# thomasdeppisch/eMagLS

Hardware: AMD Instinct MI355X
Metric: eMagLS filter sets/s (N=4, 2702 dirs, 512 taps) (higher is better)
Workload: dtype f64; 1 GPU; BASELINE config 3: getEMagLsFilters em32 r=4.2cm N=4 complex-SH, 2702 dirs, 512 taps, 48 kHz; one filter set per step, inputs resident in HBM; dirs=2702, taps=512, sim_order=19, bins=512, k_cut=43, designs_resident_per_gpu=128, designs_per_batch=32, batches_in_flight=4, distinct_hrir_sets_resident=20, parallelism=independent jobs per GPU, one RCCL gather

## Files before the change

### emagls_amd/csrc/fft.hip

```cpp
#include "kernels.hpp"
#include "lds_fft.hpp"
#include "wave_fft.hpp"

namespace emagls {

__global__ void twiddle_kernel(int nfft, cplx* __restrict__ tw, size_t bstride) {
    tw = boff(tw, bstride);
    int j = blockIdx.x * blockDim.x + threadIdx.x;
    if (j >= nfft) return;
    double s, c;
    sincos(-2.0 * kPi * (double)j / (double)nfft, &s, &c);
    if (j == 0) { c = 1.0; s = 0.0; }
    if (2 * j == nfft) { c = -1.0; s = 0.0; }
    if (4 * j == nfft) { c = 0.0; s = -1.0; }
    if (4 * j == 3 * nfft) { c = 0.0; s = 1.0; }
    tw[j] = mk(c, s);
}

__global__ void __launch_bounds__(256) hrir_dirsum_kernel(const double* __restrict__ hL, const double* __restrict__ hR,
                                                          int64_t L, int64_t D, int chunk, double* __restrict__ partial, size_t bstride) {
    hL = boff(hL, bstride); hR = boff(hR, bstride); partial = boff(partial, bstride);
    const int e = blockIdx.y;
    const double* h = e ? hR : hL;
    const int64_t d0 = (int64_t)blockIdx.x * chunk;
    const int64_t d1 = min(D, d0 + chunk);
    for (int64_t n = threadIdx.x; n < L; n += blockDim.x) {
        double acc = 0.0;
        for (int64_t d = d0; d < d1; ++d) acc += h[d * L + n];
        partial[((int64_t)blockIdx.x * 2 + e) * L + n] = acc;
    }
}

__global__ void __launch_bounds__(1024) grpdelay_median_kernel(const double* __restrict__ partial, int nchunks, int64_t L,
                                                               int nfft, const cplx* __restrict__ tw,
                                                               double* __restrict__ grpd, size_t bstride) {
    partial = boff(partial, bstride); tw = boff(tw, bstride); grpd = boff(grpd, bstride);
    extern __shared__ __attribute__((aligned(16))) char smem[];
    double* b = reinterpret_cast<double*>(smem);
    double* v = b + ((L + 1) & ~(int64_t)1);
    const int e = blockIdx.x;
    const int P = nfft / 2 + 1;
    int npow2 = 1;
    while (npow2 < P) npow2 <<= 1;
    {
        double* part = reinterpret_cast<double*>(reinterpret_cast<cplx*>(v + npow2) + nfft);
        const int nq = (int)max((int64_t)1, min((int64_t)8, (int64_t)blockDim.x / max(L, (int64_t)1)));
        for (int64_t idx = threadIdx.x; idx < (int64_t)nq * L; idx += blockDim.x) {
            const int64_t n = idx % L;
            const int q = (int)(idx / L);
            double a0 = 0.0, a1 = 0.0, a2 = 0.0, a3 = 0.0;
            int c = q;
            for (; c + 3 * nq < nchunks; c += 4 * nq) {
                a0 += partial[((int64_t)c * 2 + e) * L + n];
                a1 += partial[((int64_t)(c + nq) * 2 + e) * L + n];
                a2 += partial[((int64_t)(c + 2 * nq) * 2 + e) * L + n];
                a3 += partial[((int64_t)(c + 3 * nq) * 2 + e) * L + n];
            }
            for (; c < nchunks; c += nq) a0 += partial[((int64_t)c * 2 + e) * L + n];
            part[idx] = (a0 + a1) + (a2 + a3);
        }
        __syncthreads();
        for (int64_t n = threadIdx.x; n < L; n += blockDim.x) {
            double acc = 0.0;
            for (int q = 0; q < nq; ++q) acc += part[(int64_t)q * L + n];
            b[n] = acc;
        }
    }
    __syncthreads();
    cplx* tws = reinterpret_cast<cplx*>(v + npow2);
    for (int j = threadIdx.x; j < nfft; j += blockDim.x) tws[j] = tw[j];
    __syncthreads();
    auto finish = [](cplx num, cplx den) {
        if (cabs(den) < 10.0 * 2.220446049250313e-16) { num = mk(0, 0); den = mk(1, 0); }
        return cdiv(num, den).x;
    };
    const int kmain = min(P, (int)blockDim.x);
    for (int k = threadIdx.x; k < npow2; k += blockDim.x) v[k] = INFINITY;
    if ((int)threadIdx.x < kmain) {
        const int k = threadIdx.x;
        cplx num = mk(0, 0), den = mk(0, 0);
        int j = 0;
        for (int64_t n = 0; n < L; ++n) {
            const cplx w = tws[j];
            j += k; if (j >= nfft) j -= nfft;
            cfma(den, b[n], w);
            cfma(num, (double)n * b[n], w);
        }
        v[k] = finish(num, den);
    }
    for (int k = kmain; k < P; ++k) {
        __shared__ double red[16];
        cplx num = mk(0, 0), den = mk(0, 0);
        for (int64_t n = threadIdx.x; n < L; n += blockDim.x) {
            const cplx w = tws[(int)(((int64_t)k * n) % nfft)];
            cfma(den, b[n], w);
            cfma(num, (double)n * b[n], w);
        }
        double parts[4] = {num.x, num.y, den.x, den.y};
        for (int q = 0; q < 4; ++q) {
            double x = wave_sum(parts[q]);
            __syncthreads();
            if ((threadIdx.x & 63) == 0) red[threadIdx.x >> 6] = x;
            __syncthreads();
            double t = 0.0;
            for (int w = 0; w < (int)(blockDim.x >> 6); ++w) t += red[w];
            parts[q] = t;
        }
        if (threadIdx.x == 0) v[k] = finish(mk(parts[0], parts[1]), mk(parts[2], parts[3]));
    }
    __syncthreads();
    for (int size = 2; size <= npow2; size <<= 1) {
        for (int stride = size >> 1; stride > 0; stride >>= 1) {
            for (int i = threadIdx.x; i < npow2 / 2; i += blockDim.x) {
                const int lo = ((i / stride) * 2 * stride) + (i % stride);
                const int hi = lo + stride;
                const bool up = ((lo & size) == 0);
                const double a = v[lo], c = v[hi];
                if ((a > c) == up) { v[lo] = c; v[hi] = a; }
            }
            __syncthreads();
        }
    }
    const double med = (P & 1) ? v[(P - 1) / 2] : 0.5 * (v[P / 2 - 1] + v[P / 2]);
    if (threadIdx.x == 0) grpd[e] = med;
    cplx* phs = reinterpret_cast<cplx*>(grpd + 2) + (size_t)e * P;
    for (int kb = threadIdx.x; kb < P; kb += blockDim.x) {
        double sn, cs;
        sincos((6.283185307179586 * ((double)kb / (double)nfft)) * med, &sn, &cs);
        if (kb == P - 1) sn = 0.0;
        phs[kb] = mk(cs, sn);
    }
}

constexpr int HF_TD = 8;
constexpr int HF_MAXS = 3;
template <int TS>
__global__ void __launch_bounds__(512) hrir_fft_kernel(const double* __restrict__ hL, const double* __restrict__ hR,
                                                       int64_t L, int64_t D, const int64_t* __restrict__ didx, int nfft,
                                                       int log2n,
                                                       const cplx* __restrict__ tw, const double* __restrict__ grpd,
                                                       int mode, int n_c, int kabs0, cplx* __restrict__ Hc,
                                                       double* __restrict__ Habs, int64_t ldD, double* __restrict__ HcT, int ldT,
                                                       size_t bstride) {
    hL = boff(hL, bstride); hR = boff(hR, bstride); didx = boff(didx, bstride); tw = boff(tw, bstride); grpd = boff(grpd, bstride); Hc = boff(Hc, bstride); Habs = boff(Habs, bstride);
    HcT = boff(HcT, bstride);
    extern __shared__ __attribute__((aligned(16))) char smem[];
    const int P = nfft / 2 + 1;
    cplx* tws = reinterpret_cast<cplx*>(smem);
    cplx* phs = tws;
    cplx* buf = tws + 2 * P;
    const int64_t d0 = (int64_t)blockIdx.x * HF_TD;
    const int nt = (int)min((int64_t)HF_TD, D - d0);
// ... 47 lines not shown
            if (kb < P) {
#pragma unroll
                for (int t = 0; t < TS; ++t) {
                    if (t < nts) {
                        const cplx* x = buf + (size_t)t * nfft;
                        const cplx z = x[kb], zc = conj(x[(nfft - kb) & (nfft - 1)]);
                        cplx HLv = mk(0.5 * (z.x + zc.x), 0.5 * (z.y + zc.y));
                        cplx HRv = mk(0.5 * (z.y - zc.y), -0.5 * (z.x - zc.x));
                        if (mode == 0) {
                            HLv = HLv * phs[kb];
                            HRv = HRv * phs[P + kb];
                        }
                        if (!live[2 * (t0 + t)]) HLv = mk(0.0, 0.0);
                        if (!live[2 * (t0 + t) + 1]) HRv = mk(0.0, 0.0);
                        const int64_t d = d0 + t0 + t;
                        if (kb < n_c) {
                            Hc[((int64_t)0 * n_c + kb) * ldD + d] = HLv;
                            Hc[((int64_t)1 * n_c + kb) * ldD + d] = HRv;
                        }
                        const double nl2 = norm2(HLv), nr2 = norm2(HRv);
                        habs[s][0][t0 + t] = nl2 > 0.0 ? nl2 * fast_rsqrt(nl2) : 0.0;
                        habs[s][1][t0 + t] = nr2 > 0.0 ? nr2 * fast_rsqrt(nr2) : 0.0;
                    }
                }
            }
        }
        if (HcT) {
            for (int idx = threadIdx.x; idx < TS * n_c; idx += blockDim.x) {
                const int t = idx / n_c, kb = idx - t * n_c;
                if (t >= nts) continue;
                const cplx* x = buf + (size_t)t * nfft;
                const cplx z = x[kb], zc = conj(x[(nfft - kb) & (nfft - 1)]);
                cplx HLv = mk(0.5 * (z.x + zc.x), 0.5 * (z.y + zc.y));
                cplx HRv = mk(0.5 * (z.y - zc.y), -0.5 * (z.x - zc.x));
                if (mode == 0) { HLv = HLv * phs[kb]; HRv = HRv * phs[P + kb]; }
                if (!live[2 * (t0 + t)]) HLv = mk(0.0, 0.0);
                if (!live[2 * (t0 + t) + 1]) HRv = mk(0.0, 0.0);
                double* row = HcT + (int64_t)(d0 + t0 + t) * ldT;
                row[2 * kb] = HLv.x; row[2 * kb + 1] = HLv.y;
                row[2 * (n_c + kb)] = HRv.x; row[2 * (n_c + kb) + 1] = HRv.y;
            }
        }
    }
    const int64_t na = P - kabs0;
#pragma unroll
    for (int s = 0; s < HF_MAXS; ++s) {
        const int kb = threadIdx.x + s * 512;
        if (kb < P && kb >= kabs0) {
#pragma unroll
            for (int e = 0; e < 2; ++e) {
                double* row = Habs + ((int64_t)e * na + (kb - kabs0)) * ldD + d0;
                if (nt == HF_TD) {
#pragma unroll
                    for (int t = 0; t < HF_TD; t += 2) *reinterpret_cast<double2*>(row + t) = make_double2(habs[s][e][t], habs[s][e][t + 1]);
                } else {
#pragma unroll
                    for (int t = 0; t < HF_TD; ++t) if (t < nt) row[t] = habs[s][e][t];
                }
            }
        }
    }
}

constexpr int HW_TD = 8;
constexpr int HW_STRIDE = WF_BUF + 1;
__global__ void __launch_bounds__(64 * HW_TD) hrir_fft_wave_kernel(const double* __restrict__ hL, const double* __restrict__ hR,
                                                                   int64_t L, int64_t D, const int64_t* __restrict__ didx,
                                                                   const cplx* __restrict__ tw, const double* __restrict__ grpd,
                                                                   int mode, int n_c, int kabs0, cplx* __restrict__ Hc,
                                                                   double* __restrict__ Habs, int64_t ldD, double* __restrict__ HcT, int ldT,
                                                                   size_t bstride) {
    hL = boff(hL, bstride); hR = boff(hR, bstride); didx = boff(didx, bstride); tw = boff(tw, bstride); grpd = boff(grpd, bstride); Hc = boff(Hc, bstride); Habs = boff(Habs, bstride);
    HcT = boff(HcT, bstride);
    extern __shared__ __attribute__((aligned(16))) char smem[];
    constexpr int P = WF_N / 2 + 1;
    cplx* tables = reinterpret_cast<cplx*>(smem);
    cplx* bufs = tables + WF_TABLES;
    const int tid = threadIdx.x, w = tid >> 6, l = tid & 63;
    wave_fft_tables(tables, tw, tid, 64 * HW_TD);
    __syncthreads();
    const int64_t d0 = (int64_t)blockIdx.x * HW_TD;
    const int nt = (int)min((int64_t)HW_TD, D - d0);
    cplx* tb = bufs + (size_t)w * HW_STRIDE;
    if (w < nt) {
        const int64_t d = d0 + w;
        const int64_t dsrc = didx ? didx[d] : d;
        const double* pl = hL + dsrc * L;
        const double* pr = hR + dsrc * L;
        cplx v[16];
        const bool upper_zero = mode == 0 && L <= WF_N / 2;
        if (mode == 0) {
#pragma unroll
            for (int n1 = 0; n1 < 16; ++n1) {
                const int n = 64 * n1 + l;
                v[n1] = (n < L && (n1 < 8 || !upper_zero)) ? mk(pl[n], pr[n]) : mk(0.0, 0.0);
            }
        } else {
            const int sL = (int)round(grpd[0]), sR = (int)round(grpd[1]);
#pragma unroll
            for (int n1 = 0; n1 < 16; ++n1) {
                const int n = 64 * n1 + l;
                int nl = (n + sL) % WF_N; if (nl < 0) nl += WF_N;
                int nr = (n + sR) % WF_N; if (nr < 0) nr += WF_N;
                v[n1] = mk(nl < L ? pl[nl] : 0.0, nr < L ? pr[nr] : 0.0);
            }
        }
        bool nzL = false, nzR = false;
#pragma unroll
        for (int n1 = 0; n1 < 16; ++n1) { nzL |= v[n1].x != 0.0; nzR |= v[n1].y != 0.0; }
        const bool liveL = __any(nzL), liveR = __any(nzR);
        if (upper_zero) wave_fft1024<true>(v, tb, tables, l); else wave_fft1024<false>(v, tb, tables, l);
        wave_fft_store_natural(v, tb, l);
        wave_lds_fence();
        const cplx* phs = reinterpret_cast<const cplx*>(grpd + 2);
#pragma unroll
        for (int s = 0; s < 9; ++s) {
            const int kb = l + 64 * s;
            if (kb < P) {
                const cplx z = tb[wf_slot(kb)], zc = conj(tb[wf_slot((WF_N - kb) & (WF_N - 1))]);
                cplx HLv = mk(0.5 * (z.x + zc.x), 0.5 * (z.y + zc.y));
                cplx HRv = mk(0.5 * (z.y - zc.y), -0.5 * (z.x - zc.x));
                if (mode == 0) {
                    HLv = HLv * phs[kb];
                    HRv = HRv * phs[P + kb];
                }
                if (!liveL) HLv = mk(0.0, 0.0);
                if (!liveR) HRv = mk(0.0, 0.0);
                if (kb < n_c) {
                    Hc[((int64_t)0 * n_c + kb) * ldD + d] = HLv;
                    Hc[((int64_t)1 * n_c + kb) * ldD + d] = HRv;
                    if (HcT) {
                        double* rowT = HcT + d * ldT;
                        *reinterpret_cast<cplx*>(rowT + 2 * kb) = HLv;
                        *reinterpret_cast<cplx*>(rowT + 2 * (n_c + kb)) = HRv;
                    }
                }
                const double nl2 = norm2(HLv), nr2 = norm2(HRv);
                tb[wf_slot(kb)] = mk(nl2 > 0.0 ? nl2 * fast_rsqrt(nl2) : 0.0, nr2 > 0.0 ? nr2 * fast_rsqrt(nr2) : 0.0);
            }
        }
    }
    __syncthreads();
    const int64_t na = P - kabs0;
    const int t = tid & (HW_TD - 1);
    if (t < nt) {
        const double* src = reinterpret_cast<const double*>(bufs + (size_t)t * HW_STRIDE);
        for (int idx = tid >> 3; idx < 2 * (P - kabs0); idx += 64) {
            const int e = idx >= P - kabs0, kr = idx - e * (P - kabs0);
            Habs[((int64_t)e * na + kr) * ldD + d0 + t] = src[2 * wf_slot(kr + kabs0) + e];
        }
    }
}

__global__ void __launch_bounds__(512) real_fft_gather_kernel(const double* __restrict__ x, int64_t L, int64_t ncols,
                                                              const int64_t* __restrict__ colidx, int nfft, int log2n,
                                                              int TP, const cplx* __restrict__ tw,
                                                              cplx* __restrict__ out, int64_t ldo, int64_t inner,
                                                              int64_t ld_inner) {
    extern __shared__ __attribute__((aligned(16))) char smem[];
    cplx* tws = reinterpret_cast<cplx*>(smem);
    cplx* buf = tws + nfft / 2;
    const int P = nfft / 2 + 1;
    const int64_t p0 = (int64_t)blockIdx.x * TP;
    const int64_t npairs = (ncols + 1) / 2;
    const int nt = (int)min((int64_t)TP, npairs - p0);
    for (int j = threadIdx.x; j < nfft / 2; j += blockDim.x) tws[j] = tw[j];
    for (int idx = threadIdx.x; idx < nt * nfft; idx += blockDim.x) {
        const int t = idx / nfft, n = idx - t * nfft;
        const int64_t j0 = 2 * (p0 + t), j1 = j0 + 1;
        double a = 0.0, c = 0.0;
        if (n < L) {
            a = x[(colidx ? colidx[j0] : j0) * L + n];
            if (j1 < ncols) c = x[(colidx ? colidx[j1] : j1) * L + n];
        }
        buf[(size_t)t * nfft + bitrev((unsigned)n, log2n)] = mk(a, c);
    }
    __syncthreads();
    lds_fft_stages<false>(buf, tws, nfft, log2n, nt);
    for (int idx = threadIdx.x; idx < P * 2 * TP; idx += blockDim.x) {
        const int kb = idx / (2 * TP), r = idx - kb * 2 * TP;
        const int t = r >> 1, which = r & 1;
        if (t >= nt) continue;
        const int64_t j = 2 * (p0 + t) + which;
        if (j >= ncols) continue;
        const cplx* xx = buf + (size_t)t * nfft;
        const cplx z = xx[kb], zc = conj(xx[(nfft - kb) & (nfft - 1)]);
        out[(int64_t)kb * ldo + (j / inner) * ld_inner + (j % inner)] = which ? mk(0.5 * (z.y - zc.y), -0.5 * (z.x - zc.x))
                                           : mk(0.5 * (z.x + zc.x), 0.5 * (z.y + zc.y));
    }
}

__global__ void __launch_bounds__(256) filter_epilogue_kernel(const cplx* __restrict__ W, int C, int nfft, int log2n,
                                                              int len, const cplx* __restrict__ tw,
                                                              const double* __restrict__ grpd, int conj_mode,
                                                              int dc_rule, int shift_mode, int out_cplx, double fade_rel,
                                                              void* __restrict__ outL, void* __restrict__ outR, size_t bstride) {
    W = boff(W, bstride); tw = boff(tw, bstride); grpd = boff(grpd, bstride); outL = boff(outL, bstride); outR = boff(outR, bstride);
    extern __shared__ __attribute__((aligned(16))) char smem[];
    cplx* tws = reinterpret_cast<cplx*>(smem);
    cplx* buf = tws + nfft / 2;
    const int c = blockIdx.x, e = blockIdx.y;
    const int P = nfft / 2 + 1;
    const cplx* We = W + (size_t)e * P * C;
    for (int j = threadIdx.x; j < nfft / 2; j += blockDim.x) tws[j] = tw[j];
    int cpart = c;
    double sgn = 1.0;
    if (conj_mode == 1) {
        const int n = (int)floor(sqrt((double)c));
        const int m = c - n * n - n;
        cpart = n * n + n - m;
        sgn = (m & 1) ? -1.0 : 1.0;
    } else if (conj_mode == 2) {
        cpart = (c == 0) ? 0 : ((c & 1) ? c + 1 : c - 1);
    }
    const int n_shift = nfft / 2;
    const double delay = (e == 0) ? (double)n_shift : ((double)n_shift + grpd[1]) - grpd[0];
    for (int k = threadIdx.x; k < nfft; k += blockDim.x) {
        cplx v;
        int kb;
        if (k < P) {
            kb = k;
            v = We[(size_t)kb * C + c];
            if (kb == 0 && dc_rule) v = mk(We[(size_t)1 * C + c].x, 0.0);
        } else {
            kb = nfft - k;
            v = conj(We[(size_t)kb * C + cpart]);
            v.x *= sgn; v.y *= sgn;
        }
        if (shift_mode == 0) {
            const double omega = (double)kb / (double)nfft;
            double s, cs;
            sincos((6.283185307179586 * omega) * delay, &s, &cs);
            cplx E = mk(cs, -s);
            if (kb == P - 1) E.y = 0.0;
            if (k >= P) E.y = -E.y;
            v = v * E;
        }
        buf[bitrev((unsigned)k, log2n)] = v;
    }
    __syncthreads();
    lds_fft_stages<true>(buf, tws, nfft, log2n, 1);
    const double inv_n = 1.0 / (double)nfft;
    const int nf = (int)round(fade_rel * (double)len);
    const int t0 = n_shift - len / 2;
    for (int tt = threadIdx.x; tt < len; tt += blockDim.x) {
        int t = t0 + tt;
        if (shift_mode == 1) { t = (t - n_shift) % nfft; if (t < 0) t += nfft; }
        cplx v = buf[t];
        double win = 1.0;
        if (tt < nf || tt >= len - nf) {
            int i = (tt < nf) ? tt : (2 * nf - 1 - (nf + (tt - (len - nf))));
            win = 0.5 - 0.5 * cos(2.0 * kPi * (double)i / (double)(2 * nf - 1));
        }
        v.x *= inv_n * win;
        v.y *= inv_n * win;
        if (out_cplx) {
            cplx* o = reinterpret_cast<cplx*>(e ? outR : outL);
            o[(size_t)c * len + tt] = v;
        } else {
            double* o = reinterpret_cast<double*>(e ? outR : outL);
            o[(size_t)c * len + tt] = v.x;
        }
    }
}

constexpr int HD_TD = 8;
__global__ void __launch_bounds__(256) hrir_dft_kernel(const double* __restrict__ hL, const double* __restrict__ hR, int64_t L, int64_t D,
                                                       const int64_t* __restrict__ didx, int nfft, const cplx* __restrict__ tw,
                                                       const double* __restrict__ grpd, int mode, int n_c, int kabs0, cplx* __restrict__ Hc,
                                                       double* __restrict__ Habs, int64_t ldD, double* __restrict__ HcT, int ldT, int td, size_t bstride) {
    hL = boff(hL, bstride); hR = boff(hR, bstride); didx = boff(didx, bstride); tw = boff(tw, bstride); grpd = boff(grpd, bstride);
    Hc = boff(Hc, bstride); Habs = boff(Habs, bstride); HcT = boff(HcT, bstride);
    extern __shared__ __attribute__((aligned(16))) char smem[];
    double* hs = reinterpret_cast<double*>(smem);
    const int P = nfft / 2 + 1;
    const int64_t d0 = (int64_t)blockIdx.x * td;
    const int nt = (int)min((int64_t)td, D - d0);
    for (int64_t idx = threadIdx.x; idx < (int64_t)nt * 2 * L; idx += blockDim.x) {
        const int t = (int)(idx / (2 * L)), e = (int)((idx / L) & 1);
        const int64_t n = idx % L;
        const int64_t dsrc = didx ? didx[d0 + t] : d0 + t;
        hs[idx] = (e ? hR : hL)[dsrc * L + n];
    }
    __syncthreads();
    const double g[2] = {grpd[0], grpd[1]};
    const int64_t na = P - kabs0;
    for (int kb = threadIdx.x; kb < P; kb += blockDim.x) {
        cplx ph[2];
        for (int e = 0; e < 2; ++e) {
            if (mode == 0) {
                double sn, cs;
                sincos((6.283185307179586 * ((double)kb / (double)nfft)) * g[e], &sn, &cs);
                if (kb == P - 1) sn = 0.0;
                ph[e] = mk(cs, sn);
            } else {
                const int64_t sft = (int64_t)round(g[e]);
                int64_t j = (-(int64_t)kb * sft) % nfft;
                if (j < 0) j += nfft;
                ph[e] = tw[j];
            }
        }
        for (int t = 0; t < nt; ++t) {
            cplx H[2] = {mk(0.0, 0.0), mk(0.0, 0.0)};
            const double* h0 = hs + (int64_t)t * 2 * L;
            int j = 0;
            for (int64_t n = 0; n < L; ++n) {
                const cplx w = tw[j];
                cfma(H[0], h0[n], w); cfma(H[1], h0[L + n], w);
                j += kb; if (j >= nfft) j -= nfft;
            }
            const int64_t d = d0 + t;
            for (int e = 0; e < 2; ++e) {
                const cplx v = H[e] * ph[e];
                if (kb < n_c) {
                    Hc[((int64_t)e * n_c + kb) * ldD + d] = v;
                    if (HcT) { double* row = HcT + d * ldT; row[2 * (e * n_c + kb)] = v.x; row[2 * (e * n_c + kb) + 1] = v.y; }
                }
                if (kb >= kabs0) Habs[((int64_t)e * na + (kb - kabs0)) * ldD + d] = sqrt(norm2(v));
            }
        }
    }
}

__global__ void __launch_bounds__(256) real_dft_gather_kernel(const double* __restrict__ x, int64_t L, int64_t ncols, const int64_t* __restrict__ colidx,
                                                              int nfft, const cplx* __restrict__ tw, cplx* __restrict__ out, int64_t ldo, int64_t inner,
                                                              int64_t ld_inner) {
    extern __shared__ __attribute__((aligned(16))) char smem[];
    double* xs = reinterpret_cast<double*>(smem);
    const int64_t j = blockIdx.x;
    const int P = nfft / 2 + 1;
    const double* col = x + (colidx ? colidx[j] : j) * L;
    for (int64_t n = threadIdx.x; n < L; n += blockDim.x) xs[n] = col[n];
    __syncthreads();
    for (int kb = threadIdx.x; kb < P; kb += blockDim.x) {
        cplx acc = mk(0.0, 0.0);
        int jj = 0;
        for (int64_t n = 0; n < L && n < nfft; ++n) { cfma(acc, xs[n], tw[jj]); jj += kb; if (jj >= nfft) jj -= nfft; }
        out[(int64_t)kb * ldo + (j / inner) * ld_inner + (j % inner)] = acc;
    }
}

__global__ void __launch_bounds__(256) filter_epilogue_dft_kernel(const cplx* __restrict__ W, int C, int nfft, int len, const cplx* __restrict__ tw,
                                                                  const double* __restrict__ grpd, int conj_mode, int dc_rule, int shift_mode, int out_cplx,
                                                                  double fade_rel, void* __restrict__ outL, void* __restrict__ outR, size_t bstride) {
    W = boff(W, bstride); tw = boff(tw, bstride); grpd = boff(grpd, bstride); outL = boff(outL, bstride); outR = boff(outR, bstride);
    extern __shared__ __attribute__((aligned(16))) char smem[];
    cplx* buf = reinterpret_cast<cplx*>(smem);
    const int c = blockIdx.x, e = blockIdx.y;
    const int P = nfft / 2 + 1;
    const cplx* We = W + (size_t)e * P * C;
    int cpart = c;
    double sgn = 1.0;
    if (conj_mode == 1) {
        const int n = (int)floor(sqrt((double)c));
        const int m = c - n * n - n;
        cpart = n * n + n - m;
        sgn = (m & 1) ? -1.0 : 1.0;
    } else if (conj_mode == 2) {
        cpart = (c == 0) ? 0 : ((c & 1) ? c + 1 : c - 1);
    }
    const int n_shift = nfft / 2;
    const double delay = (e == 0) ? (double)n_shift : ((double)n_shift + grpd[1]) - grpd[0];
    for (int k = threadIdx.x; k < nfft; k += blockDim.x) {
        cplx v;
        int kb;
        if (k < P) {
            kb = k;
            v = We[(size_t)kb * C + c];
            if (kb == 0 && dc_rule) v = mk(We[(size_t)1 * C + c].x, 0.0);
        } else {
            kb = nfft - k;
            v = conj(We[(size_t)kb * C + cpart]);
            v.x *= sgn; v.y *= sgn;
        }
        if (shift_mode == 0) {
            const double omega = (double)kb / (double)nfft;
            double sn, cs;
            sincos((6.283185307179586 * omega) * delay, &sn, &cs);
            cplx E = mk(cs, -sn);
            if (kb == P - 1) E.y = 0.0;
            if (k >= P) E.y = -E.y;
            v = v * E;
        }
        buf[k] = v;
    }
    __syncthreads();
    const double inv_n = 1.0 / (double)nfft;
    const int nf = (int)round(fade_rel * (double)len);
    const int t0 = n_shift - len / 2;
    for (int tt = threadIdx.x; tt < len; tt += blockDim.x) {
        int t = t0 + tt;
        if (shift_mode == 1) { t = (t - n_shift) % nfft; if (t < 0) t += nfft; }
        cplx v = mk(0.0, 0.0);
        int j = 0;
        for (int k = 0; k < nfft; ++k) { cfma(v, buf[k], conj(tw[j])); j += t; if (j >= nfft) j -= nfft; }
        double win = 1.0;
        if (tt < nf || tt >= len - nf) {
            int i = (tt < nf) ? tt : (2 * nf - 1 - (nf + (tt - (len - nf))));
            win = 0.5 - 0.5 * cos(2.0 * kPi * (double)i / (double)(2 * nf - 1));
        }
        v.x *= inv_n * win;
        v.y *= inv_n * win;
        if (out_cplx) reinterpret_cast<cplx*>(e ? outR : outL)[(size_t)c * len + tt] = v;
        else reinterpret_cast<double*>(e ? outR : outL)[(size_t)c * len + tt] = v.x;
    }
}

static int ilog2(int n) { int l = 0; while ((1 << l) < n) ++l; return l; }
static bool is_pow2(int n) { return n > 0 && (n & (n - 1)) == 0; }

void launch_twiddles(int nfft, void* tw, hipStream_t st) {
    twiddle_kernel<<<bgrid((nfft + 255) / 256), 256, 0, st>>>(nfft, (cplx*)tw, batch_ctx().stride);
    KERNEL_CHECK();
}

int hrir_dirsum_chunks(int64_t D) { return (int)ceil_div(D, 64); }

void launch_hrir_grpdelay(const double* hL, const double* hR, int64_t L, int64_t D, int nfft, const void* tw,
                          double* partial, double* grpd, hipStream_t st) {
    const int chunk = 64;
    const int nchunks = hrir_dirsum_chunks(D);
    hrir_dirsum_kernel<<<bgrid(dim3(nchunks, 2)), 256, 0, st>>>(hL, hR, L, D, chunk, partial, batch_ctx().stride);
    KERNEL_CHECK();
    const int P = nfft / 2 + 1;
    int npow2 = 1;
    while (npow2 < P) npow2 <<= 1;
    size_t sm = (((size_t)L + 1) & ~(size_t)1) * 8 + (size_t)npow2 * 8 + (size_t)nfft * 16 + (size_t)std::max<int64_t>(1024, L) * 8;
    static PerDeviceOnce median_once;
    if (median_once.first()) HIP_CHECK(hipFuncSetAttribute((const void*)grpdelay_median_kernel, hipFuncAttributeMaxDynamicSharedMemorySize, 128 * 1024));
    grpdelay_median_kernel<<<bgrid(2), 1024, sm, st>>>(partial, nchunks, L, nfft, (const cplx*)tw, grpd, batch_ctx().stride);
    KERNEL_CHECK();
}

void launch_hrir_fft(const double* hL, const double* hR, int64_t L, int64_t D, const int64_t* didx, int nfft,
                     const void* tw, const double* grpd, int mode, int n_c, int kabs0, void* Hc, double* Habs,
                     int64_t ldD, hipStream_t st, double* HcT, int ldT) {
    if (!is_pow2(nfft)) {
        int td = HD_TD;
        while (td > 1 && (size_t)td * 2 * L * 8 > 48 * 1024) td >>= 1;
        if ((size_t)td * 2 * L * 8 > 64 * 1024) throw Error(2, "HRIR DFT: more than 4096 taps is not supported");
        hrir_dft_kernel<<<bgrid((unsigned)ceil_div(D, td)), 256, (size_t)td * 2 * L * 8, st>>>(hL, hR, L, D, didx, nfft, (const cplx*)tw, grpd, mode, n_c, kabs0,
                                                                                                (cplx*)Hc, Habs, ldD, HcT, ldT, td, batch_ctx().stride);
        KERNEL_CHECK();
        return;
    }
    const int log2n = ilog2(nfft);
    const int P = nfft / 2 + 1;
    if (P > HF_MAXS * 512) throw Error(2, "HRIR FFT: nfft above 2048 is not supported");
    if (nfft == WF_N && L <= WF_N && sw_on<Sw::HRIR_FFT_WAVE>()) {
        const size_t smw = sizeof(cplx) * (WF_TABLES + (size_t)HW_TD * HW_STRIDE);
        static PerDeviceOnce wave_once;
        if (wave_once.first())
            HIP_CHECK(hipFuncSetAttribute((const void*)hrir_fft_wave_kernel, hipFuncAttributeMaxDynamicSharedMemorySize, 160 * 1024));
        hrir_fft_wave_kernel<<<bgrid((unsigned)ceil_div(D, HW_TD)), 64 * HW_TD, smw, st>>>(hL, hR, L, D, didx, (const cplx*)tw, grpd, mode, n_c, kabs0,
                                                                                      (cplx*)Hc, Habs, ldD, HcT, ldT, batch_ctx().stride);
        KERNEL_CHECK();
        return;
    }
    size_t budget = (nfft >= 2048 ? 110 : 83) * 1024;
    if (const int kb = sw_int<Sw::HRIR_FFT_LDS_KB>()) budget = (size_t)kb * 1024;
    const size_t shared = (size_t)2 * P * 16 + 2 * HF_TD * sizeof(int);
    int TS = HF_TD;
    while (TS > 1 && (size_t)TS * nfft * 16 + shared > budget) TS >>= 1;
    const size_t sm = (size_t)TS * nfft * 16 + shared;
    static PerDeviceOnce attr_once;
    if (attr_once.first()) {
        HIP_CHECK(hipFuncSetAttribute((const void*)hrir_fft_kernel<8>, hipFuncAttributeMaxDynamicSharedMemorySize, 160 * 1024));
        HIP_CHECK(hipFuncSetAttribute((const void*)hrir_fft_kernel<4>, hipFuncAttributeMaxDynamicSharedMemorySize, 160 * 1024));
        HIP_CHECK(hipFuncSetAttribute((const void*)hrir_fft_kernel<2>, hipFuncAttributeMaxDynamicSharedMemorySize, 160 * 1024));
        HIP_CHECK(hipFuncSetAttribute((const void*)hrir_fft_kernel<1>, hipFuncAttributeMaxDynamicSharedMemorySize, 160 * 1024));
        HIP_CHECK(hipFuncSetAttribute((const void*)real_fft_gather_kernel, hipFuncAttributeMaxDynamicSharedMemorySize, 160 * 1024));
    }
    const dim3 grid = bgrid((unsigned)ceil_div(D, HF_TD));
#define EMAGLS_HF(TSV)                                                                                                               \
    hrir_fft_kernel<TSV><<<grid, 512, sm, st>>>(hL, hR, L, D, didx, nfft, log2n, (const cplx*)tw, grpd, mode, n_c, kabs0, (cplx*)Hc, \
                                                Habs, ldD, HcT, ldT, batch_ctx().stride)
    switch (TS) {
        case 8: EMAGLS_HF(8); break;
        case 4: EMAGLS_HF(4); break;
        case 2: EMAGLS_HF(2); break;
        default: EMAGLS_HF(1); break;
    }
#undef EMAGLS_HF
    KERNEL_CHECK();
}

void launch_real_fft_gather(const double* x, int64_t L, int64_t ncols, const int64_t* colidx, int nfft, const void* tw,
                            void* out, int64_t ldo, int64_t inner, int64_t ld_inner, hipStream_t st) {
    if (!is_pow2(nfft)) {
        if ((size_t)L * 8 > 64 * 1024) throw Error(2, "ATF DFT: more than 8192 taps is not supported");
        real_dft_gather_kernel<<<(unsigned)ncols, 256, (size_t)L * 8, st>>>(x, L, ncols, colidx, nfft, (const cplx*)tw, (cplx*)out, ldo, inner, ld_inner);
        KERNEL_CHECK();
        return;
    }
    const int log2n = ilog2(nfft);
    int TP = 8;
    while (TP > 1 && (size_t)TP * nfft * 16 + (size_t)nfft * 8 > 150 * 1024) TP >>= 1;
    const size_t sm = (size_t)TP * nfft * 16 + (size_t)nfft * 8;
    static PerDeviceOnce attr_once;
    if (attr_once.first()) {
        HIP_CHECK(hipFuncSetAttribute((const void*)real_fft_gather_kernel, hipFuncAttributeMaxDynamicSharedMemorySize, 160 * 1024));
    }
    const int64_t npairs = (ncols + 1) / 2;
    real_fft_gather_kernel<<<(unsigned)ceil_div(npairs, TP), 512, sm, st>>>(x, L, ncols, colidx, nfft, log2n, TP,
                                                                          (const cplx*)tw, (cplx*)out, ldo, inner, ld_inner);
    KERNEL_CHECK();
}

void launch_filter_epilogue(const void* W, int C, int nfft, int len, const void* tw, const double* grpd, int conj_mode,
                            int dc_rule, int shift_mode, int out_cplx, void* outL, void* outR, hipStream_t st, int n_ears,
                            double fade_rel) {
    if (!is_pow2(nfft)) {
        const size_t smd = (size_t)nfft * 16;
        if (smd > 64 * 1024) throw Error(2, "filter epilogue: a non-power-of-two FFT length above 4096 is not supported");
        filter_epilogue_dft_kernel<<<bgrid(dim3(C, n_ears)), 256, smd, st>>>((const cplx*)W, C, nfft, len, (const cplx*)tw, grpd, conj_mode, dc_rule, shift_mode,
                                                                           out_cplx, fade_rel, outL, outR, batch_ctx().stride);
        KERNEL_CHECK();
        return;
    }
    const int log2n = ilog2(nfft);
    const size_t sm = (size_t)nfft * 16 + (size_t)nfft * 8;
    if (sm > 48 * 1024) {
        static PerDeviceOnce attr_once;
        if (attr_once.first()) {
            HIP_CHECK(hipFuncSetAttribute((const void*)filter_epilogue_kernel, hipFuncAttributeMaxDynamicSharedMemorySize, 160 * 1024));
        }
    }
    filter_epilogue_kernel<<<bgrid(dim3(C, n_ears)), 256, sm, st>>>((const cplx*)W, C, nfft, log2n, len, (const cplx*)tw, grpd,
                                                        conj_mode, dc_rule, shift_mode, out_cplx, fade_rel, outL, outR, batch_ctx().stride);
    KERNEL_CHECK();
}

}
```

### emagls_amd/csrc/switches.hpp

```cpp
#pragma once
#include <climits>
#include <cmath>

namespace emagls {

#define EMAGLS_SWITCHES(X) \
    X(PLAN_CACHE,        INT,  4,     0, INT_MAX,   PROCESS, "shapes the one-shot entry points keep alive (0 = off)") \
    X(BATCH_MAX,         INT,  8,     1, 32,        PROCESS, "initial limit of designs per batch, read at load time (emagls_set_batch_max changes it at run time; the job scheduler sets it per chunk)") \
    X(BATCH_GROUPS,      INT,  2,     1, 4,         CALL,    "lane groups of a batch of more than 8 designs before its sweep (1 = one launch sequence)") \
    X(BATCH_LANES,       ON0,  1,     0, 1,         CALL,    "=0: batches in stream mode (per-plan pipelines) instead of lane mode") \
    X(DEBUG_LANES,       ON1,  0,     0, 1,         CALL,    "=1: why a batch was refused lane mode or common routes, on stderr") \
    X(STAGGER,           ON0,  1,     0, 1,         PROCESS, "=0: both lane groups of a batch issue the stages before the sweep in one order (default: complementary orders)") \
    X(DEFER_HH,          INT,  1,     0, 2,         PROCESS, "the orthonormal route of the low bins next to the sweep: 0 never, 1 batches and designs that have the device to themselves, 2 every lane batch") \
    X(GEO_KEEP,          ON0,  1,     0, 1,         PROCESS, "=0: sharing batches run their geometry stages on every execute") \
    X(GEO_LS_SHARED,     ON0,  1,     0, 1,         CALL,    "=0: sharing batches carry every HRIR set's least-squares rows through the factors instead of one kept Y_reg_inv per bin") \
    X(GRAM_LDS,          ON0,  1,     0, 1,         PROCESS, "=0: lane batches take the K-split Gram kernel + reduce instead of the LDS-staged one") \
    X(GRAM_MFMA4,        ON1,  0,     0, 1,         CALL,    "=1: the Gram tile on the 4 x 4 x 4 MFMA shape (measured slower; the tests' second form)") \
    X(XCD_RUNS,          ON0,  1,     0, 1,         PROCESS, "=0: gram_lds, gemm_tn_f64, synth_ls take their tiles in dispatch order instead of XCD-aware runs") \
    X(GRAM_ROUTE,        ON0,  1,     0, 1,         CALL,    "=0: no Gram route (all bins Householder + Jacobi)") \
    X(GRAM_COND_EST,     REAL, 3e3,   -HUGE_VAL, HUGE_VAL, CALL, "conditioning estimate below which the Gram route starts (the device check stays at 3e4)") \
    X(JACOBI_RUN,        INT,  0,     1, INT_MAX,   PROCESS, "bins per Jacobi workgroup on the Gram route (0: single bins where the stages are forked, runs of 2 in lane groups)") \
    X(REAL_INTERNAL,     ON0,  1,     0, 1,         CALL,    "=0: complex-basis eMagLS / eMagLS2 designs on the complex-arithmetic pipeline") \
    X(NO_GRAPH,          ON1,  0,     0, 1,         CALL,    "=1: eager launches instead of hipGraph replay (plans and batches, when they are created)") \
    X(STREAMS,           INT,  0,     1, 4,         CALL,    "streams of a single plan (0: one, until emagls_plan_set_streams)") \
    X(ONESHOT_STREAMS,   INT,  1,     1, 3,         CALL,    "streams of the one-shot plans of array designs") \
    X(SWEEP_PERSIST,     ON0,  1,     0, 1,         CALL,    "=0: launch-per-bin sweep instead of the persistent one") \
    X(PERSIST_GLOBAL,    ON1,  0,     0, 1,         CALL,    "=1: write-through granules even when a design sits on one XCD") \
    X(SWEEP_SYNTH,       ON0,  1,     0, 1,         CALL,    "=0: array designs on materialised operands instead of the synthesising sweep (when a plan is created)") \
    X(SWEEP_TWIN,        ON0,  1,     0, 1,         CALL,    "=0: launches of 9-16 designs as two independent workgroups per CU instead of twin workgroups") \
    X(SWEEP_REG,         INT,  1,     0, 2,         CALL,    "register-resident sweep: 0 never (the slab form), 1 for launches of more than 8 designs, 2 always") \
    X(REG_WAVES,         INT,  0,     INT_MIN, INT_MAX, CALL, "waves per workgroup of the register-resident sweep (4, 6, 8, 10, 12 whenever it fits; 0: the smallest count with which every workgroup owns a CU)") \
    X(REG_SPREAD,        INT,  2,     0, 2,         CALL,    "a launch's designs spread over all XCDs: 0 never, 1 whenever it fits, 2 when it needs fewer waves per workgroup than the one-XCD layout") \
    X(REG_PRIO,          INT,  1,     INT_MIN, INT_MAX, PROCESS, "=0: the register-resident sweep's waves at the default issue priority") \
    X(SWEEP_FETCH,       INT,  0,     0, 4,         PROCESS, "where the persistent sweep requests the next bin's operands") \
    X(SWEEP_WAIT_MS,     INT,  20,    1, INT_MAX,   PROCESS, "wall-clock limit of a wait for peers inside a resident sweep, in ms") \
    X(SWEEP_TIMING,      ON1,  0,     0, 1,         CALL,    "=1: in-kernel wall-clock stamps of the persistent sweep (when a plan is created)") \
    X(CU_BUDGET,         INT,  0,     0, INT_MAX,   CALL,    "CUs the resident sweeps may count on when their residency is decided (0: the device's)") \
    X(SYNTH_PAIRS,       ON0,  1,     0, 1,         PROCESS, "=0: synthesising sweep without antipodal microphone pairs") \
    X(SYNTH_SPLIT,       INT,  67,    INT_MIN, INT_MAX, PROCESS, "synthesising sweep: per cent of the producers' unit groups evaluated before barrier B1") \
    X(SYNTH_PRIO,        INT,  5,     0, 5,         PROCESS, "synthesising sweep: issue priorities (5: the chains of the two designs of an XCD tilted against the age order; 0: all chains 3, producers 0)") \
    X(STREAM_POOL,       ON0,  1,     0, 1,         PROCESS, "=0: destroy streams instead of recycling them (exposes a HIP runtime crash in long sessions)") \
    X(STREAM_WARM,       INT,  8,     0, INT_MAX,   PROCESS, "streams the pool parks before it hands the first one out") \
    X(POOL_GB,           INT,  128,   0, INT_MAX,   PROCESS, "device memory the block pool keeps for the next plans and arenas, in GB") \
    X(JOBS_FORK,         INT,  3,     1, 4,         PROCESS, "job scheduler: streams of a job list that is a single chunk (1 = lane groups as for chunks in flight)") \
    X(JOBS_RESIDENT,     INT,  0,     0, INT_MAX,   CALL,    "job scheduler: designs whose plans and batches stay resident between calls (0: max(256, 2 x batch x in flight))") \
    X(JOBS_AUTO_SHARE,   ON0,  1,     0, 1,         PROCESS, "=0: job scheduler shares no geometry unless the caller asks") \
    X(JOBS_TRACE,        ON1,  0,     0, 1,         PROCESS, "=1: time stamps of every chunk's steps and of block pool misses on stderr") \
    X(HRIR_FFT_WAVE,     ON0,  1,     0, 1,         CALL,    "=0: the HRIR prologue at nfft = 1024 on the LDS radix-2^2 transform instead of wave-private transforms") \
    X(HRIR_FFT_LDS_KB,   INT,  0,     40, 158,      CALL,    "LDS budget of the LDS-form HRIR transform's sub-tiles (0: 83, 110 at nfft = 2048)") \
    X(DECODE_FUSED,      ON0,  1,     0, 1,         CALL,    "=0: binauralDecode on the hipFFT passes for every filter length") \
    X(DECODE_REGFFT,     ON0,  1,     0, 1,         CALL,    "=0: the fused decode kernel on LDS transform passes also up to 512 taps") \
    X(DECODE_WAVE,       ON0,  1,     0, 1,         CALL,    "=0: the half-wave two-factor decode form also at 257-512 taps") \
    X(DECODE_FILTER_FFT, ONH,  0,     0, 1,         CALL,    "=hipfft: the filter side of the decode's wave form through hipFFT") \
    X(WA_REG,            ON0,  1,     0, 1,         CALL,    "=0: the 33-64-channel path's Householder kernels walk the columns through L2") \
    X(WA_TALL,           ON0,  1,     0, 1,         CALL,    "=0: the plain Householder kernels for problems of more than 448 rows instead of the LDS-reflector forms") \
    X(WA_YRI_MFMA,       ON0,  1,     0, 1,         CALL,    "=0: the 33-64-channel path's Y_reg_inv_k product on the vector pipe") \
    X(WA_JACOBI_FLAG,    REAL, 1e-14, -HUGE_VAL, HUGE_VAL, PROCESS, "the 33-64-channel path's Jacobi: another sweep follows one in which some rotation had |gamma| > x sqrt(alpha beta)") \
    X(WA_LEAF_ROWS,      INT,  0,     INT_MIN, INT_MAX, PROCESS, "tiled QR: upper bound of the leaf height, 1024 .. 4096 (anything else: 3072)")

enum class Sw : int {
#define X(name, kind, def, lo, hi, when, doc) name,
    EMAGLS_SWITCHES(X)
#undef X
    COUNT
};
enum class SwKind { ON0, ON1, ONH, INT, REAL };
constexpr SwKind sw_kind(Sw s) {
    constexpr SwKind kinds[] = {
#define X(name, kind, def, lo, hi, when, doc) SwKind::kind,
        EMAGLS_SWITCHES(X)
#undef X
    };
    return kinds[(int)s];
}

double sw_value(Sw s);

template <Sw S> inline bool sw_on() {
    static_assert(sw_kind(S) == SwKind::ON0 || sw_kind(S) == SwKind::ON1 || sw_kind(S) == SwKind::ONH, "not a flag");
    return sw_value(S) != 0.0;
}
template <Sw S> inline int sw_int() { static_assert(sw_kind(S) == SwKind::INT, "not an integer switch"); return (int)sw_value(S); }
template <Sw S> inline double sw_real() { static_assert(sw_kind(S) == SwKind::REAL, "not a real switch"); return sw_value(S); }

}
```

### emagls_amd/csrc/wave_fft.hpp

```cpp
#pragma once
#include "reg_fft.hpp"

namespace emagls {

constexpr int WF_N = 1024;
constexpr int WF_ROW = 68;
constexpr int WF_BUF = 16 * WF_ROW;
constexpr int WF_TW1 = 1024;
constexpr int WF_TW2 = 64;
constexpr int WF_TABLES = WF_TW1 + WF_TW2;

__host__ __device__ constexpr int wf_bin(int l, int i) { return (l >> 2) + 16 * ((l & 3) + 4 * (i >> 3)) + 128 * rf_bitrev<3>(i & 7); }
__host__ __device__ constexpr int wf_slot(int k) { return (k & ~7) | ((k + 2 * ((k >> 4) & 3)) & 7); }

__device__ __forceinline__ void wave_fft_tables(cplx* tables, const cplx* __restrict__ circle, int tid, int nthreads) {
    for (int idx = tid; idx < WF_TW1; idx += nthreads) tables[idx] = circle[(idx & 63) * rf_bitrev<4>(idx >> 6)];
    for (int idx = tid; idx < WF_TW2; idx += nthreads) {
        const int d = idx >> 5, j = (idx >> 2) & 7, s = idx & 3;
        tables[WF_TW1 + idx] = circle[16 * ((s + 4 * d) * rf_bitrev<3>(j))];
    }
}

__device__ __forceinline__ void wave_lds_fence() {
    __builtin_amdgcn_fence(__ATOMIC_RELEASE, "wavefront");
    __builtin_amdgcn_wave_barrier();
    __builtin_amdgcn_fence(__ATOMIC_ACQUIRE, "wavefront");
}

__device__ __forceinline__ void reg_fft16_upper_zero(cplx (&v)[16]) {
    constexpr double C16[8] = {1.0, 0.9238795325112867, 0.7071067811865476, 0.38268343236508984, 0.0, -0.3826834323650897,
                               -0.7071067811865475, -0.9238795325112867};
    constexpr double S16[8] = {0.0, -0.3826834323650898, -0.7071067811865475, -0.9238795325112867, -1.0, -0.9238795325112867,
                               -0.7071067811865476, -0.3826834323650899};
#pragma unroll
    for (int i = 0; i < 8; ++i) {
        const cplx a = v[i];
        if (i == 0) v[8] = a;
        else if (i == 4) v[12] = mk(a.y, -a.x);
        else v[8 + i] = mk(a.x * C16[i] - a.y * S16[i], a.x * S16[i] + a.y * C16[i]);
    }
    cplx lo[8], hi[8];
#pragma unroll
    for (int i = 0; i < 8; ++i) { lo[i] = v[i]; hi[i] = v[8 + i]; }
    reg_fft<8>(lo);
    reg_fft<8>(hi);
#pragma unroll
    for (int i = 0; i < 8; ++i) { v[i] = lo[i]; v[8 + i] = hi[i]; }
}

template <bool UPPER_ZERO>
__device__ __forceinline__ void wf_pass1(cplx (&v)[16], cplx* tb, const cplx* tables, int l) {
    if (UPPER_ZERO) reg_fft16_upper_zero(v); else reg_fft<16>(v);
    const int lsw = (l & ~7) | ((l + (l >> 3)) & 7);
#pragma unroll
    for (int i0 = 0; i0 < 16; i0 += 4) {
        cplx t[4];
#pragma unroll
        for (int i = 0; i < 4; ++i) t[i] = tables[(i0 + i) * 64 + l];
#pragma unroll
        for (int i = 0; i < 4; ++i) tb[rf_bitrev<4>(i0 + i) * WF_ROW + lsw] = v[i0 + i] * t[i];
        __builtin_amdgcn_sched_barrier(0);
    }
    wave_lds_fence();
}
template <int H>
__device__ __forceinline__ void wf_pass2_half(cplx* tb, const cplx* tables, int l) {
    const int b = (l & 3) + 4 * H;
    cplx* row = tb + (l >> 2) * WF_ROW;
    const cplx* tw2 = tables + WF_TW1 + 32 * H + (l & 3);
    cplx u[8];
#pragma unroll
    for (int a = 0; a < 8; ++a) u[a] = row[8 * a + ((b + a) & 7)];
    reg_fft<8>(u);
#pragma unroll
    for (int j = 0; j < 8; ++j) {
        const int ka = rf_bitrev<3>(j);
        row[8 * ka + ((b + ka) & 7)] = (j == 0) ? u[j] : u[j] * tw2[4 * j];
    }
}
template <int E>
__device__ __forceinline__ void wf_pass3_half(cplx (&out)[8], const cplx* tb, int l) {
    const int ka = (l & 3) + 4 * E;
    const cplx* rowk = tb + (l >> 2) * WF_ROW + 8 * ka;
#pragma unroll
    for (int b = 0; b < 8; ++b) out[b] = rowk[(b + ka) & 7];
    reg_fft<8>(out);
}

template <bool UPPER_ZERO>
__device__ __forceinline__ void wave_fft1024(cplx (&v)[16], cplx* tb, const cplx* tables, int l) {
    wf_pass1<UPPER_ZERO>(v, tb, tables, l);
    wf_pass2_half<0>(tb, tables, l);
    wf_pass2_half<1>(tb, tables, l);
    wave_lds_fence();
    cplx u0[8], u1[8];
    wf_pass3_half<0>(u0, tb, l);
    wf_pass3_half<1>(u1, tb, l);
    wave_lds_fence();
#pragma unroll
    for (int j = 0; j < 8; ++j) { v[j] = u0[j]; v[8 + j] = u1[j]; }
}

__device__ __forceinline__ void wave_fft_store_natural(const cplx (&v)[16], cplx* tb, int l) {
    const int base = (l >> 2) + 16 * (l & 3);
#pragma unroll
    for (int i = 0; i < 16; ++i) tb[wf_slot(base + 64 * (i >> 3) + 128 * rf_bitrev<3>(i & 7))] = v[i];
}

}
```

Measured before the change: 4384 filter sets/s.

## Add persistent tile-loop HRIR wave FFT kernel with prefetch, pruning and LDS staging

Adds a persistent-workgroup version of the wave-private 1024-point HRIR FFT. Each workgroup loops over direction tiles, sized to eight workgroups per CU, and prefetches the next tile's taps into registers while the current one transforms. The first register radix-16 stage is pruned to the number of nonzero input rows, and the complex bins below n_c are staged in LDS so they can be written out coalesced. This cuts launch-tail and global load latency and skips zero arithmetic, at the cost of more register pressure and extra LDS traffic; the new form becomes the default.

```diff
diff --git a/emagls_amd/csrc/fft.hip b/emagls_amd/csrc/fft.hip
--- a/emagls_amd/csrc/fft.hip
+++ b/emagls_amd/csrc/fft.hip
@@ -1,3 +1,5 @@
+#include <atomic>
+
 #include "kernels.hpp"
 #include "lds_fft.hpp"
 #include "wave_fft.hpp"
@@ -351,6 +353,169 @@
     }
 }
 
+constexpr int HW_NC_STAGED = 248;
+constexpr int HW_STAGE0 = 520;
+constexpr int HW_WGS_PER_CU = 8;
+template <int NZ, int MODE>
+__global__ void __launch_bounds__(64 * HW_TD) hrir_fft_wave_tiles_kernel(const double* __restrict__ hL, const double* __restrict__ hR,
+                                                                         int64_t L, int64_t D, const int64_t* __restrict__ didx,
+                                                                         const cplx* __restrict__ tw, const double* __restrict__ grpd,
+                                                                         int n_c, int kabs0, cplx* __restrict__ Hc,
+                                                                         double* __restrict__ Habs, int64_t ldD, double* __restrict__ HcT, int ldT,
+                                                                         size_t bstride) {
+    hL = boff(hL, bstride); hR = boff(hR, bstride); didx = boff(didx, bstride); tw = boff(tw, bstride); grpd = boff(grpd, bstride); Hc = boff(Hc, bstride); Habs = boff(Habs, bstride);
+    HcT = boff(HcT, bstride);
+    extern __shared__ __attribute__((aligned(16))) char smem[];
+    constexpr int P = WF_N / 2 + 1;
+    constexpr bool AHEAD = NZ <= 2;
+    cplx* tables = reinterpret_cast<cplx*>(smem);
+    cplx* bufs = tables + WF_TABLES;
+    const int tid = threadIdx.x, w = tid >> 6, l = tid & 63;
+    wave_fft_tables(tables, tw, tid, 64 * HW_TD);
+    __syncthreads();
+    cplx* tb = bufs + (size_t)w * HW_STRIDE;
+    const int64_t ntiles = (D + HW_TD - 1) / HW_TD;
+    const bool staged = n_c <= HW_NC_STAGED;
+    const cplx* phs = reinterpret_cast<const cplx*>(grpd + 2);
+    const int64_t na = P - kabs0;
+    int sL = 0, sR = 0;
+    if (MODE != 0) { sL = (int)round(grpd[0]); sR = (int)round(grpd[1]); }
+    auto load_taps = [&](cplx (&x)[NZ], int64_t d, int l) {
+        const int64_t dsrc = didx ? didx[d] : d;
+        const double* pl = hL + dsrc * L;
+        const double* pr = hR + dsrc * L;
+        if (MODE == 0) {
+#pragma unroll
+            for (int n1 = 0; n1 < NZ; ++n1) {
+                const int n = 64 * n1 + l;
+                x[n1] = n < L ? mk(pl[n], pr[n]) : mk(0.0, 0.0);
+            }
+        } else {
+#pragma unroll
+            for (int n1 = 0; n1 < NZ; ++n1) {
+                const int n = 64 * n1 + l;
+                int nl = (n + sL) % WF_N; if (nl < 0) nl += WF_N;
+                int nr = (n + sR) % WF_N; if (nr < 0) nr += WF_N;
+                x[n1] = mk(nl < L ? pl[nl] : 0.0, nr < L ? pr[nr] : 0.0);
+            }
+        }
+    };
+    auto live_ears = [&](const cplx (&x)[NZ], bool& liveL, bool& liveR) {
+        bool nzL = false, nzR = false;
+#pragma unroll
+        for (int n1 = 0; n1 < NZ; ++n1) { nzL |= x[n1].x != 0.0; nzR |= x[n1].y != 0.0; }
+        liveL = __any(nzL); liveR = __any(nzR);
+    };
+    cplx x[NZ];
+    bool liveL = false, liveR = false;
+    int64_t tile = blockIdx.x;
+    if constexpr (AHEAD) {
+        if (tile * HW_TD + w < D) {
+            load_taps(x, tile * HW_TD + w, l);
+            live_ears(x, liveL, liveR);
+        }
+    }
+    for (; tile < ntiles; tile += gridDim.x) {
+        const int64_t d0 = tile * HW_TD;
+        const int nt = (int)min((int64_t)HW_TD, D - d0);
+        const int64_t d = d0 + w;
+        const bool have = w < nt;
+        bool hasL = liveL, hasR = liveR;
+        int lt = l;
+        asm volatile("" : "+v"(lt));
+        cplx v[16];
+        if (have) {
+            if constexpr (AHEAD) {
+#pragma unroll
+                for (int n1 = 0; n1 < NZ; ++n1) v[n1] = x[n1];
+            } else {
+                cplx y[NZ];
+                load_taps(y, d, lt);
+                live_ears(y, hasL, hasR);
+#pragma unroll
+                for (int n1 = 0; n1 < NZ; ++n1) v[n1] = y[n1];
+            }
+#pragma unroll
+            for (int n1 = NZ; n1 < 16; ++n1) v[n1] = mk(0.0, 0.0);
+        }
+        const int64_t dn = d + (int64_t)gridDim.x * HW_TD;
+        if constexpr (AHEAD) { if (dn < D) load_taps(x, dn, lt); }
+        if (have) {
+            wave_fft1024_rows<NZ>(v, tb, tables, lt);
+            wave_fft_store_natural(v, tb, lt);
+            wave_lds_fence();
+            __builtin_amdgcn_sched_barrier(0);
+#pragma unroll
+            for (int g = 2; g >= 0; --g) {
+                cplx pL[3], pR[3], z[3], zc[3];
+#pragma unroll
+                for (int j = 0; j < 3; ++j) {
+                    const int kc = min(lt + 64 * (3 * g + 2 - j), P - 1);
+                    if (MODE == 0) { pL[j] = phs[kc]; pR[j] = phs[P + kc]; }
+                    z[j] = tb[wf_slot(kc)];
+                    zc[j] = conj(tb[wf_slot((WF_N - kc) & (WF_N - 1))]);
+                }
+#pragma unroll
+                for (int j = 0; j < 3; ++j) {
+                    const int kb = lt + 64 * (3 * g + 2 - j);
+                    if (kb < P) {
+                        cplx HLv = mk(0.5 * (z[j].x + zc[j].x), 0.5 * (z[j].y + zc[j].y));
+                        cplx HRv = mk(0.5 * (z[j].y - zc[j].y), -0.5 * (z[j].x - zc[j].x));
+                        if (MODE == 0) {
+                            HLv = HLv * pL[j];
+                            HRv = HRv * pR[j];
+                        }
+                        if (!hasL) HLv = mk(0.0, 0.0);
+                        if (!hasR) HRv = mk(0.0, 0.0);
+                        if (kb < n_c) {
+                            if (staged) {
+                                cplx* st = tb + HW_STAGE0 + 2 * (n_c - 1 - kb);
+                                st[0] = HLv;
+                                st[1] = HRv;
+                            } else {
+                                Hc[((int64_t)0 * n_c + kb) * ldD + d] = HLv;
+                                Hc[((int64_t)1 * n_c + kb) * ldD + d] = HRv;
+                                if (HcT) {
+                                    double* rowT = HcT + d * ldT;
+                                    *reinterpret_cast<cplx*>(rowT + 2 * kb) = HLv;
+                                    *reinterpret_cast<cplx*>(rowT + 2 * (n_c + kb)) = HRv;
+                                }
+                            }
+                        }
+                        const double nl2 = norm2(HLv), nr2 = norm2(HRv);
+                        tb[wf_slot(kb)] = mk(nl2 > 0.0 ? nl2 * fast_rsqrt(nl2) : 0.0, nr2 > 0.0 ? nr2 * fast_rsqrt(nr2) : 0.0);
+                    }
+                }
+            }
+        }
+        if constexpr (AHEAD) { if (dn < D) live_ears(x, liveL, liveR); }
+        __syncthreads();
+        const int t = tid & (HW_TD - 1);
+        if (t < nt) {
+            const cplx* srcc = bufs + (size_t)t * HW_STRIDE;
+            if (staged) {
+                for (int idx = tid >> 3; idx < 2 * n_c; idx += 64) {
+                    const int e = idx >= n_c, kb = idx - e * n_c;
+                    Hc[((int64_t)e * n_c + kb) * ldD + d0 + t] = srcc[HW_STAGE0 + 2 * (n_c - 1 - kb) + e];
+                }
+            }
+            const double* src = reinterpret_cast<const double*>(srcc);
+            for (int idx = tid >> 3; idx < 2 * (P - kabs0); idx += 64) {
+                const int e = idx >= P - kabs0, kr = idx - e * (P - kabs0);
+                Habs[((int64_t)e * na + kr) * ldD + d0 + t] = src[2 * wf_slot(kr + kabs0) + e];
+            }
+        }
+        if (staged && HcT) {
+            for (int idx = tid; idx < nt * 2 * n_c; idx += 64 * HW_TD) {
+                const int tt = idx / (2 * n_c), j = idx - tt * 2 * n_c;
+                const int e = j >= n_c, kb = j - e * n_c;
+                *reinterpret_cast<cplx*>(HcT + (d0 + tt) * ldT + 2 * j) = bufs[(size_t)tt * HW_STRIDE + HW_STAGE0 + 2 * (n_c - 1 - kb) + e];
+            }
+        }
+        __syncthreads();
+    }
+}
+
 __global__ void __launch_bounds__(512) real_fft_gather_kernel(const double* __restrict__ x, int64_t L, int64_t ncols,
                                                               const int64_t* __restrict__ colidx, int nfft, int log2n,
                                                               int TP, const cplx* __restrict__ tw,
@@ -607,6 +772,17 @@
 
 static int ilog2(int n) { int l = 0; while ((1 << l) < n) ++l; return l; }
 static bool is_pow2(int n) { return n > 0 && (n & (n - 1)) == 0; }
+static int device_cus() {
+    static std::atomic<int> cus[64];
+    int dev = 0;
+    HIP_CHECK(hipGetDevice(&dev));
+    int n = cus[dev & 63].load(std::memory_order_relaxed);
+    if (n <= 0) {
+        HIP_CHECK(hipDeviceGetAttribute(&n, hipDeviceAttributeMultiprocessorCount, dev));
+        cus[dev & 63].store(n, std::memory_order_relaxed);
+    }
+    return n;
+}
 
 void launch_twiddles(int nfft, void* tw, hipStream_t st) {
     twiddle_kernel<<<bgrid((nfft + 255) / 256), 256, 0, st>>>(nfft, (cplx*)tw, batch_ctx().stride);
@@ -646,11 +822,34 @@
     const int log2n = ilog2(nfft);
     const int P = nfft / 2 + 1;
     if (P > HF_MAXS * 512) throw Error(2, "HRIR FFT: nfft above 2048 is not supported");
-    if (nfft == WF_N && L <= WF_N && sw_on<Sw::HRIR_FFT_WAVE>()) {
+    const int wave_form = sw_int<Sw::HRIR_FFT_WAVE>();
+    if (nfft == WF_N && L <= WF_N && wave_form != 0) {
         const size_t smw = sizeof(cplx) * (WF_TABLES + (size_t)HW_TD * HW_STRIDE);
         static PerDeviceOnce wave_once;
-        if (wave_once.first())
+        if (wave_once.first()) {
             HIP_CHECK(hipFuncSetAttribute((const void*)hrir_fft_wave_kernel, hipFuncAttributeMaxDynamicSharedMemorySize, 160 * 1024));
+            HIP_CHECK(hipFuncSetAttribute((const void*)hrir_fft_wave_tiles_kernel<2, 0>, hipFuncAttributeMaxDynamicSharedMemorySize, 160 * 1024));
+            HIP_CHECK(hipFuncSetAttribute((const void*)hrir_fft_wave_tiles_kernel<8, 0>, hipFuncAttributeMaxDynamicSharedMemorySize, 160 * 1024));
+            HIP_CHECK(hipFuncSetAttribute((const void*)hrir_fft_wave_tiles_kernel<16, 0>, hipFuncAttributeMaxDynamicSharedMemorySize, 160 * 1024));
+            HIP_CHECK(hipFuncSetAttribute((const void*)hrir_fft_wave_tiles_kernel<16, 1>, hipFuncAttributeMaxDynamicSharedMemorySize, 160 * 1024));
+        }
+        if (wave_form == 2) {
+            const int64_t tiles = ceil_div(D, HW_TD);
+            int64_t wgs = sw_int<Sw::HRIR_FFT_WGS>();
+            if (wgs <= 0) wgs = std::max(1, (HW_WGS_PER_CU * device_cus() + batch_ctx().n - 1) / batch_ctx().n);
+            const dim3 grid = bgrid((unsigned)std::min(tiles, wgs));
+            const int rows = (int)ceil_div(L, 64);
+#define EMAGLS_HW(NZ, MODE)                                                                                                             \
+    hrir_fft_wave_tiles_kernel<NZ, MODE><<<grid, 64 * HW_TD, smw, st>>>(hL, hR, L, D, didx, (const cplx*)tw, grpd, n_c, kabs0, (cplx*)Hc, \
+                                                                        Habs, ldD, HcT, ldT, batch_ctx().stride)
+            if (mode != 0) EMAGLS_HW(16, 1);
+            else if (rows <= 2) EMAGLS_HW(2, 0);
+            else if (rows <= 8) EMAGLS_HW(8, 0);
+            else EMAGLS_HW(16, 0);
+#undef EMAGLS_HW
+            KERNEL_CHECK();
+            return;
+        }
         hrir_fft_wave_kernel<<<bgrid((unsigned)ceil_div(D, HW_TD)), 64 * HW_TD, smw, st>>>(hL, hR, L, D, didx, (const cplx*)tw, grpd, mode, n_c, kabs0,
                                                                                       (cplx*)Hc, Habs, ldD, HcT, ldT, batch_ctx().stride);
         KERNEL_CHECK();
diff --git a/emagls_amd/csrc/switches.hpp b/emagls_amd/csrc/switches.hpp
--- a/emagls_amd/csrc/switches.hpp
+++ b/emagls_amd/csrc/switches.hpp
@@ -46,7 +46,8 @@
     X(JOBS_RESIDENT,     INT,  0,     0, INT_MAX,   CALL,    "job scheduler: designs whose plans and batches stay resident between calls (0: max(256, 2 x batch x in flight))") \
     X(JOBS_AUTO_SHARE,   ON0,  1,     0, 1,         PROCESS, "=0: job scheduler shares no geometry unless the caller asks") \
     X(JOBS_TRACE,        ON1,  0,     0, 1,         PROCESS, "=1: time stamps of every chunk's steps and of block pool misses on stderr") \
-    X(HRIR_FFT_WAVE,     ON0,  1,     0, 1,         CALL,    "=0: the HRIR prologue at nfft = 1024 on the LDS radix-2^2 transform instead of wave-private transforms") \
+    X(HRIR_FFT_WAVE,     INT,  2,     0, 2,         CALL,    "the HRIR prologue at nfft = 1024: 2 wave-private transforms with the tiles in a loop, 1 one workgroup per tile (the form before it), 0 the LDS radix-2^2 transform") \
+    X(HRIR_FFT_WGS,      INT,  0,     0, 65535,     CALL,    "workgroups per lane of the HRIR prologue's tile loop (0: eight per CU over all lanes of the launch)") \
     X(HRIR_FFT_LDS_KB,   INT,  0,     40, 158,      CALL,    "LDS budget of the LDS-form HRIR transform's sub-tiles (0: 83, 110 at nfft = 2048)") \
     X(DECODE_FUSED,      ON0,  1,     0, 1,         CALL,    "=0: binauralDecode on the hipFFT passes for every filter length") \
     X(DECODE_REGFFT,     ON0,  1,     0, 1,         CALL,    "=0: the fused decode kernel on LDS transform passes also up to 512 taps") \
diff --git a/emagls_amd/csrc/wave_fft.hpp b/emagls_amd/csrc/wave_fft.hpp
--- a/emagls_amd/csrc/wave_fft.hpp
+++ b/emagls_amd/csrc/wave_fft.hpp
@@ -48,9 +48,39 @@
     for (int i = 0; i < 8; ++i) { v[i] = lo[i]; v[8 + i] = hi[i]; }
 }
 
-template <bool UPPER_ZERO>
-__device__ __forceinline__ void wf_pass1(cplx (&v)[16], cplx* tb, const cplx* tables, int l) {
-    if (UPPER_ZERO) reg_fft16_upper_zero(v); else reg_fft<16>(v);
+template <int NZ> __device__ __forceinline__ void reg_fft16_rows(cplx (&v)[16]) {
+    static_assert(NZ == 2 || NZ == 4 || NZ == 8 || NZ == 16, "rows of the pruned register stage");
+    constexpr double C32[16] = {1.0, 0.9807852804032304, 0.9238795325112867, 0.8314696123025452, 0.7071067811865476, 0.5555702330196023,
+                                0.38268343236508984, 0.19509032201612833, 0.0, -0.1950903220161282, -0.3826834323650897, -0.555570233019602,
+                                -0.7071067811865475, -0.8314696123025453, -0.9238795325112867, -0.9807852804032304};
+    constexpr double S32[16] = {0.0, -0.19509032201612825, -0.3826834323650898, -0.5555702330196022, -0.7071067811865475, -0.8314696123025452,
+                                -0.9238795325112867, -0.9807852804032304, -1.0, -0.9807852804032304, -0.9238795325112867, -0.8314696123025455,
+                                -0.7071067811865476, -0.5555702330196022, -0.3826834323650899, -0.1950903220161286};
+#pragma unroll
+    for (int span = 8; span >= 1; span >>= 1) {
+#pragma unroll
+        for (int i = 0; i < 16; ++i) {
+            if ((i & span) == 0) {
+                const int j = i + span;
+                const int k = (i & (span - 1)) * (16 / span);
+                const cplx a = v[i];
+                double tx = a.x, ty = a.y;
+                if (span < NZ) {
+                    const cplx b = v[j];
+                    v[i] = mk(a.x + b.x, a.y + b.y);
+                    tx = a.x - b.x; ty = a.y - b.y;
+                } else if ((i & (span - 1)) >= NZ) {
+                    continue;
+                }
+                if (k == 0) v[j] = mk(tx, ty);
+                else if (k == 8) v[j] = mk(ty, -tx);
+                else v[j] = mk(tx * C32[k] - ty * S32[k], tx * S32[k] + ty * C32[k]);
+            }
+        }
+    }
+}
+
+__device__ __forceinline__ void wf_pass1_store(cplx (&v)[16], cplx* tb, const cplx* tables, int l) {
     const int lsw = (l & ~7) | ((l + (l >> 3)) & 7);
 #pragma unroll
     for (int i0 = 0; i0 < 16; i0 += 4) {
@@ -62,6 +92,16 @@
         __builtin_amdgcn_sched_barrier(0);
     }
     wave_lds_fence();
+}
+template <bool UPPER_ZERO>
+__device__ __forceinline__ void wf_pass1(cplx (&v)[16], cplx* tb, const cplx* tables, int l) {
+    if (UPPER_ZERO) reg_fft16_upper_zero(v); else reg_fft<16>(v);
+    wf_pass1_store(v, tb, tables, l);
+}
+template <int NZ>
+__device__ __forceinline__ void wf_pass1_rows(cplx (&v)[16], cplx* tb, const cplx* tables, int l) {
+    reg_fft16_rows<NZ>(v);
+    wf_pass1_store(v, tb, tables, l);
 }
 template <int H>
 __device__ __forceinline__ void wf_pass2_half(cplx* tb, const cplx* tables, int l) {
@@ -101,6 +141,20 @@
     for (int j = 0; j < 8; ++j) { v[j] = u0[j]; v[8 + j] = u1[j]; }
 }
 
+template <int NZ>
+__device__ __forceinline__ void wave_fft1024_rows(cplx (&v)[16], cplx* tb, const cplx* tables, int l) {
+    wf_pass1_rows<NZ>(v, tb, tables, l);
+    wf_pass2_half<0>(tb, tables, l);
+    wf_pass2_half<1>(tb, tables, l);
+    wave_lds_fence();
+    cplx u0[8], u1[8];
+    wf_pass3_half<0>(u0, tb, l);
+    wf_pass3_half<1>(u1, tb, l);
+    wave_lds_fence();
+#pragma unroll
+    for (int j = 0; j < 8; ++j) { v[j] = u0[j]; v[8 + j] = u1[j]; }
+}
+
 __device__ __forceinline__ void wave_fft_store_natural(const cplx (&v)[16], cplx* tb, int l) {
     const int base = (l >> 2) + 16 * (l & 3);
 #pragma unroll
```

Result: slower. 4337 filter sets/s (-1.1%).
